# delldu/MaskRCNN

Measured on AMD Instinct MI355X. Metric: images/sec at 1024x1024, 1000 proposals/img (Mask R-CNN inference hot path), higher is better.
Workload: dtype f32

## Files before the change

include/maskrcnn_hip.h:

```cpp
#ifndef MASKRCNN_HIP_H
#define MASKRCNN_HIP_H

#include <stddef.h>
#include <stdint.h>

#ifdef __cplusplus
extern "C" {
#endif

#define MRCNN_ABI_VERSION 22

#define MRCNN_OK 0
#define MRCNN_ERR_INVALID_ARGUMENT (-1)
#define MRCNN_ERR_UNSUPPORTED (-2)
#define MRCNN_ERR_LAUNCH (-3)

typedef void* mrcnn_stream_t;

int mrcnn_abi_version(void);
const char* mrcnn_last_error(void);
const char* mrcnn_arch(void);

int64_t mrcnn_nms_max_boxes(void);
size_t mrcnn_nms_workspace_bytes(int32_t num_segments, int64_t n_max);
int mrcnn_nms_batched_f32(const float* dets, int32_t num_segments, int64_t n_max, int64_t seg_stride,
                          int64_t row_stride, int64_t col_stride, const int32_t* seg_counts,
                          const int32_t* class_ids, float threshold, int64_t* keep_out,
                          int32_t* counts_out, void* workspace, size_t workspace_bytes,
                          mrcnn_stream_t stream);

size_t mrcnn_nms_general_workspace_bytes(int64_t n, int32_t dtype);
int mrcnn_nms_general(const void* dets, int32_t dtype, int64_t n, int64_t row_stride, int64_t col_stride, float threshold,
                      int64_t* keep_out, int64_t* count_out, void* workspace, size_t workspace_bytes,
                      mrcnn_stream_t stream);

int mrcnn_crop_forward_f32(const float* image, int32_t batch, int32_t depth, int32_t height,
                           int32_t width, const float* boxes, const int32_t* box_index,
                           int32_t num_boxes, float extrapolation_value, int32_t crop_height,
                           int32_t crop_width, float* crops, mrcnn_stream_t stream);

int mrcnn_crop_backward_f32(const float* grads, const float* boxes, const int32_t* box_index,
                            int32_t num_boxes, int32_t batch, int32_t depth, int32_t height,
                            int32_t width, int32_t crop_height, int32_t crop_width,
// ... 133 lines not shown
int mrcnn_nhwc_to_kblocked_f32(const float* x, int64_t pixels, int32_t channels, float* y, mrcnn_stream_t stream);
size_t mrcnn_conv3x3_winograd_workspace_bytes(int32_t batch, int32_t height, int32_t width, int32_t cin);
int mrcnn_conv3x3_winograd_nhwc_f32(const float* x, int32_t batch, int32_t height, int32_t width, int32_t cin,
                                    const float* u, int32_t cout, const float* scale, const float* shift,
                                    int32_t activation, float* y, void* workspace, size_t workspace_bytes,
                                    mrcnn_stream_t stream);

int mrcnn_stem_conv7x7_s2_nhwc_f32(const float* x, int32_t batch, int32_t height, int32_t width, const float* w,
                                   const float* scale, const float* shift, int32_t activation, float* y,
                                   mrcnn_stream_t stream);
int mrcnn_stem_conv7x7_s2_nchw_f32(const float* x_nchw, int32_t batch, int32_t height, int32_t width, const float* w,
                                   const float* scale, const float* shift, int32_t activation, float* y,
                                   mrcnn_stream_t stream);
int mrcnn_stem_conv7x7_s2_nchw_f16out(const float* x_nchw, int32_t batch, int32_t height, int32_t width, const float* w,
                                      const float* scale, const float* shift, int32_t activation, void* y_f16,
                                      mrcnn_stream_t stream);
int mrcnn_stem_conv7x7_s2_pool_f32(const float* x_nchw, int32_t batch, int32_t height, int32_t width, const float* w,
                                   const float* scale, const float* shift, float* y, mrcnn_stream_t stream);
int mrcnn_stem_conv7x7_s2_pool_f16(const float* x_nchw, int32_t batch, int32_t height, int32_t width, const float* w,
                                   const float* scale, const float* shift, void* y_f16, mrcnn_stream_t stream);

size_t mrcnn_topk_workspace_bytes(int32_t batch);
int mrcnn_topk_desc_f32(const float* scores, int32_t batch, int64_t n, int32_t k, float* top_scores, int64_t* order,
                        void* workspace, size_t workspace_bytes, mrcnn_stream_t stream);
int mrcnn_proposal_select_f32(const float* dets, const int64_t* keep, const int32_t* keep_counts, int32_t batch,
                              int32_t k, int32_t proposal_count, float image_height, float image_width, float* rois,
                              int32_t* counts, mrcnn_stream_t stream);
int mrcnn_detection_select_f32(const float* dets, const int32_t* nms_class_ids, const int64_t* class_ids,
                               const int64_t* keep, const int32_t* keep_counts, int32_t batch, int32_t rois_per_image,
                               int32_t max_instances, float image_height, float image_width, int64_t* out_class_ids,
                               float* out_scores, float* out_boxes, float* out_rois, int32_t* out_counts,
                               mrcnn_stream_t stream);

int mrcnn_nchw_to_nhwc_f32(const float* x, int32_t batch, int32_t channels, int32_t height,
                           int32_t width, int32_t channels_padded, float* y, mrcnn_stream_t stream);
int mrcnn_nhwc_to_nchw_f32(const float* x, int32_t batch, int32_t channels, int32_t height,
                           int32_t width, float* y, mrcnn_stream_t stream);

size_t mrcnn_resize_u8_workspace_bytes(int32_t n, int32_t in_h, int32_t in_w, int32_t channels, int32_t out_h,
                                       int32_t out_w);
int mrcnn_resize_bilinear_u8(const uint8_t* src, int32_t n, int32_t in_h, int32_t in_w, int32_t channels,
                             int64_t src_image_stride, int64_t src_row_stride, uint8_t* dst, int32_t out_h,
                             int32_t out_w, void* workspace, size_t workspace_bytes, mrcnn_stream_t stream);
int mrcnn_mold_image_u8(const uint8_t* src, int32_t in_h, int32_t in_w, int32_t new_h, int32_t new_w, int32_t top,
                        int32_t left, int32_t out_h, int32_t out_w, const double mean_pixel[3], float* dst,
                        void* workspace, size_t workspace_bytes, mrcnn_stream_t stream);
int mrcnn_mold_images_u8(const uint8_t* src, int32_t n, int64_t src_image_stride, int32_t in_h, int32_t in_w, int32_t new_h,
                         int32_t new_w, int32_t top, int32_t left, int32_t out_h, int32_t out_w, const double mean_pixel[3],
                         float* dst, void* workspace, size_t workspace_bytes, mrcnn_stream_t stream);
int mrcnn_paste_masks_u8(const float* masks, int64_t stride_n, int64_t stride_y, int64_t stride_x, int64_t stride_c,
                         int32_t n, int32_t mask_h, int32_t mask_w, int32_t num_classes, const int64_t* class_ids,
                         const float* boxes, int32_t height, int32_t width, int32_t on_value, uint8_t* out,
                         mrcnn_stream_t stream);
size_t mrcnn_rle_workspace_bytes(int32_t n, int32_t height, int32_t width);
int mrcnn_rle_encode_u8(const uint8_t* masks, int64_t image_stride, int64_t row_stride, int32_t n, int32_t height,
                        int32_t width, int32_t threshold, int32_t capacity, int32_t* num_runs, uint32_t* counts,
                        uint8_t* strings, int32_t* string_bytes, int32_t* areas, int32_t* bboxes, void* workspace,
                        size_t workspace_bytes, mrcnn_stream_t stream);

size_t mrcnn_rle_iou_workspace_bytes(int32_t n_dt, int32_t dt_capacity, int32_t n_gt, int32_t gt_capacity);
int mrcnn_rle_iou_f64(const int32_t* dt_num_runs, const uint32_t* dt_counts, int32_t n_dt, int32_t dt_capacity,
                      const int32_t* gt_num_runs, const uint32_t* gt_counts, int32_t n_gt, int32_t gt_capacity,
                      const uint8_t* iscrowd, const int32_t* dt_off, const int32_t* gt_off, const int64_t* out_off,
                      int32_t groups, double* out, int64_t out_len, void* workspace, size_t workspace_bytes,
                      mrcnn_stream_t stream);
int mrcnn_bbox_iou_f64(const double* dt_boxes, int32_t n_dt, const double* gt_boxes, int32_t n_gt, const uint8_t* iscrowd,
// ... 59 lines not shown
```

maskrcnn_amd/csrc/common.hpp:

```cpp
#pragma once
#include <hip/hip_runtime.h>

#include <cstdarg>
#include <cstdint>
#include <cstdio>
#include <cstdlib>

#include "maskrcnn_hip.h"

namespace mrcnn {

char* error_buffer();
int fail(int code, const char* fmt, ...);

inline hipStream_t as_stream(mrcnn_stream_t s) { return reinterpret_cast<hipStream_t>(s); }

inline int check_launch(const char* what) {
    hipError_t e = hipGetLastError();
    if (e != hipSuccess) return fail(MRCNN_ERR_LAUNCH, "%s: %s", what, hipGetErrorString(e));
    return MRCNN_OK;
}

constexpr int kWave = 64;

int ensure_dynamic_lds(const void* kernel, size_t lds_bytes, const char* who);
int device_cu_count();

inline const char* tuning_env(const char* name) {
#ifdef MRCNN_TUNING
    return getenv(name);
#else
    (void)name;
    return nullptr;
#endif
}

}

#ifdef MRCNN_SYNC_FUZZ
namespace mrcnn {
__device__ __forceinline__ void sync_fuzz_point() {
    unsigned long long t;
    unsigned r;
    asm volatile("s_memtime %0\n\t"
                 "s_getreg_b32 %1, hwreg(HW_REG_HW_ID, 4, 2)\n\t"
                 "s_waitcnt lgkmcnt(0)\n\t"
                 "s_lshl_b32 %1, %1, 1\n\t"
                 "s_add_u32 %1, %1, 3\n\t"
                 "s_lshr_b64 %0, %0, %1\n\t"
                 "s_and_b64 %0, %0, 63\n\t"
                 "1:\n\t"
                 "s_cmp_eq_u64 %0, 0\n\t"
                 "s_cbranch_scc1 2f\n\t"
                 "s_sleep 64\n\t"
                 "s_lshr_b64 %0, %0, 1\n\t"
                 "s_branch 1b\n\t"
                 "2:"
                 : "=&s"(t), "=&s"(r)
                 :
                 : "scc", "memory");
}
__device__ __forceinline__ void fuzzed_syncthreads() {
    __syncthreads();
    sync_fuzz_point();
}
}
#define MRCNN_SYNC_FUZZ_POINT() ::mrcnn::sync_fuzz_point()
#define __syncthreads() ::mrcnn::fuzzed_syncthreads()
// ... 9 lines not shown
```

maskrcnn_amd/csrc/nms.hip:

```cpp
#pragma clang fp contract(off)

#include "common.hpp"

namespace {

using u64 = unsigned long long;
using u32 = unsigned int;

struct Box {
    float y1, x1, y2, x2, area;
};

__device__ __forceinline__ bool iou_ge(const Box& i, const Box& j, float thr) {
    const float xx1 = (i.x1 < j.x1) ? j.x1 : i.x1;
    const float yy1 = (i.y1 < j.y1) ? j.y1 : i.y1;
    const float xx2 = (j.x2 < i.x2) ? j.x2 : i.x2;
    const float yy2 = (j.y2 < i.y2) ? j.y2 : i.y2;
    float tw = xx2 - xx1;
    tw = tw + 1.0f;
    float th = yy2 - yy1;
    th = th + 1.0f;
    const float w = (0.0f < tw) ? tw : 0.0f;
    const float h = (0.0f < th) ? th : 0.0f;
    const float inter = w * h;
// ... 377 lines not shown
                       col_stride, seg_counts, class_ids, thr, keep_out, counts_out);
    return mrcnn::check_launch("nms_kernel");
}

template <int CAP, int T>
int launch_sort(const float* dets, int32_t S, int64_t n_max, int64_t seg_stride, int64_t row_stride,
                int64_t col_stride, const int32_t* seg_counts, const int32_t* class_ids, NmsWs ws,
                hipStream_t stream) {
    if (int rc = mrcnn::ensure_dynamic_lds(reinterpret_cast<const void*>(nms_sort_kernel<CAP, T>), sizeof(u64) * CAP, "nms"))
        return rc;
    hipLaunchKernelGGL((nms_sort_kernel<CAP, T>), dim3(S), dim3(T), sizeof(u64) * CAP, stream, dets, n_max,
                       seg_stride, row_stride, col_stride, seg_counts, class_ids, ws);
    return mrcnn::check_launch("nms_sort_kernel");
}

size_t ws_layout(int32_t S, int64_t n_max, void* base, NmsWs* ws) {
    const int np = static_cast<int>((n_max + 63) / 64 * 64), nb = np / 64;
    size_t off = 0;
    auto take = [&](size_t bytes) { size_t o = off; off += (bytes + 255) / 256 * 256; return o; };
    const size_t o_box = take(sizeof(float4) * S * np), o_area = take(sizeof(float) * S * np);
    const size_t o_cls = take(sizeof(int) * S * np), o_idx = take(sizeof(int) * S * np);
    const size_t o_col = take(sizeof(u64) * S * np * nb);
    if (ws) {
        unsigned char* b = static_cast<unsigned char*>(base);
        ws->box = reinterpret_cast<float4*>(b + o_box);
        ws->area = reinterpret_cast<float*>(b + o_area);
        ws->cls = reinterpret_cast<int*>(b + o_cls);
        ws->idx = reinterpret_cast<int*>(b + o_idx);
        ws->col = reinterpret_cast<u64*>(b + o_col);
        ws->np = np;
        ws->nb = nb;
    }
    return off;
}

}

constexpr int64_t NMS_MAX_WS = 16384, NMS_MAX_LDS = 4096;
extern "C" int64_t mrcnn_nms_max_boxes(void) { return NMS_MAX_WS; }

extern "C" size_t mrcnn_nms_workspace_bytes(int32_t num_segments, int64_t n_max) {
    if (num_segments < 1 || n_max < 1 || n_max > NMS_MAX_WS) return 0;
    return ws_layout(num_segments, n_max, nullptr, nullptr);
}

extern "C" int mrcnn_nms_batched_f32(const float* dets, int32_t num_segments, int64_t n_max,
                                     int64_t seg_stride, int64_t row_stride, int64_t col_stride,
                                     const int32_t* seg_counts, const int32_t* class_ids,
                                     float threshold, int64_t* keep_out, int32_t* counts_out,
                                     void* workspace, size_t workspace_bytes, mrcnn_stream_t stream) {
    MRCNN_REQUIRE(dets && keep_out && counts_out, "nms: null pointer");
    MRCNN_REQUIRE(num_segments >= 1, "nms: num_segments=%d must be >= 1", num_segments);
    MRCNN_REQUIRE(n_max >= 1 && n_max <= ((workspace && n_max > 128) ? NMS_MAX_WS : NMS_MAX_LDS),
                  "nms: n_max=%lld outside [1, %lld] (%lld with a workspace)", (long long)n_max, (long long)NMS_MAX_LDS,
                  (long long)NMS_MAX_WS);
    hipStream_t s = mrcnn::as_stream(stream);
    if (workspace && n_max > 128) {
        MRCNN_REQUIRE(workspace_bytes >= mrcnn_nms_workspace_bytes(num_segments, n_max),
                      "nms: workspace too small (%zu < %zu bytes)", workspace_bytes,
                      mrcnn_nms_workspace_bytes(num_segments, n_max));
        MRCNN_REQUIRE((reinterpret_cast<uintptr_t>(workspace) & 15) == 0, "nms: workspace must be 16-byte aligned");
        NmsWs ws;
        ws_layout(num_segments, n_max, workspace, &ws);
        int rc;
        if (n_max <= 1024)
            rc = launch_sort<1024, 1024>(dets, num_segments, n_max, seg_stride, row_stride, col_stride,
// ... 9 lines not shown
                                         seg_counts, class_ids, ws, s);
        else
            rc = launch_sort<16384, 1024>(dets, num_segments, n_max, seg_stride, row_stride, col_stride,
                                          seg_counts, class_ids, ws, s);
        if (rc) return rc;
        hipLaunchKernelGGL(nms_mask_kernel, dim3(ws.nb * (ws.nb + 1) / 2, num_segments), dim3(64), 0, s, ws,
                           threshold);
        if ((rc = mrcnn::check_launch("nms_mask_kernel"))) return rc;
        const size_t tail = (ws.np + 7) / 8 * 8 + sizeof(u64) * (ws.nb + 2);
        const size_t lds_full = sizeof(u64) * ws.np * ws.nb + tail;
        if (lds_full <= 150 * 1024) {
            auto k = nms_scan_kernel<true>;
            if ((rc = mrcnn::ensure_dynamic_lds(reinterpret_cast<const void*>(k), lds_full, "nms"))) return rc;
            hipLaunchKernelGGL(k, dim3(num_segments), dim3(256), lds_full, s, ws, n_max, seg_counts, keep_out,
                               counts_out);
        } else {
            hipLaunchKernelGGL(nms_scan_kernel<false>, dim3(num_segments), dim3(256), tail, s, ws, n_max,
                               seg_counts, keep_out, counts_out);
        }
        return mrcnn::check_launch("nms_scan_kernel");
    }
    if (n_max <= 256)
        return launch<256, 256>(dets, num_segments, n_max, seg_stride, row_stride, col_stride,
                                seg_counts, class_ids, threshold, keep_out, counts_out, s);
    if (n_max <= 1024)
        return launch<1024, 1024>(dets, num_segments, n_max, seg_stride, row_stride, col_stride,
                                  seg_counts, class_ids, threshold, keep_out, counts_out, s);
    if (n_max <= 2048)
        return launch<2048, 1024>(dets, num_segments, n_max, seg_stride, row_stride, col_stride,
                                  seg_counts, class_ids, threshold, keep_out, counts_out, s);
    return launch<4096, 1024>(dets, num_segments, n_max, seg_stride, row_stride, col_stride,
                              seg_counts, class_ids, threshold, keep_out, counts_out, s);
}
```

maskrcnn_amd/csrc/select.hip:

```cpp
#include "common.hpp"

namespace {

constexpr int TOPK_THREADS = 1024;
constexpr int TOPK_WAVES = TOPK_THREADS / 64;
constexpr int SORT_CAP = 4096;

__device__ __forceinline__ uint32_t order_key(float f) {
    uint32_t u = __float_as_uint(f);
    if (f != f) u = 0x7FC00000u;
    return (u & 0x80000000u) ? ~u : (u | 0x80000000u);
}

template <typename T>
__device__ __forceinline__ void bitonic_sort_desc(T* keys, int n, int tid, int nthreads) {
    for (int k = 2; k <= n; k <<= 1) {
        for (int j = k >> 1; j > 0; j >>= 1) {
            __syncthreads();
            for (int i = tid; i < n; i += nthreads) {
                const int l = i ^ j;
                if (l > i) {
                    const T a = keys[i], b = keys[l];
                    const bool desc = (i & k) == 0;
                    if (desc ? a < b : a > b) {
// ... 398 lines not shown
        float score = 0.f;
        int64_t id = 0;
        if (ok) {
            const uint32_t idx = 0xFFFFFFFFu - static_cast<uint32_t>(e);
            box = make_float4(db[idx * 5 + 0], db[idx * 5 + 1], db[idx * 5 + 2], db[idx * 5 + 3]);
            score = db[idx * 5 + 4];
            id = class_ids[static_cast<int64_t>(b) * p + idx];
        }
        out_ids[o] = id;
        out_scores[o] = score;
        reinterpret_cast<float4*>(out_boxes)[o] = box;
        reinterpret_cast<float4*>(out_rois)[o] =
            make_float4(box.x / norm_h, box.y / norm_w, box.z / norm_h, box.w / norm_w);
        return ok;
    };
    int cnt = 0;
    if (p <= 1024) {
        const uint64_t v = sort1024_desc(key_of(tid), sh.keys, tid);
        if (tid < d) cnt += emit(tid, v);
    } else {
        for (int i = tid; i < pp; i += 1024) sh.keys[i] = key_of(i);
        bitonic_sort_desc(sh.keys, pp, tid, 1024);
        for (int i = tid; i < d; i += 1024) cnt += emit(i, sh.keys[i]);
    }
    __syncthreads();
    uint32_t* total = sh.kept;
    if (tid == 0) total[0] = 0;
    __syncthreads();
    if (cnt) atomicAdd(&total[0], static_cast<uint32_t>(cnt));
    __syncthreads();
    if (tid == 0) out_counts[b] = static_cast<int32_t>(total[0]);
}

}

static size_t topk_layout(int batch, TopkWorkspace* ws, unsigned char* base) {
    auto up = [](size_t v) { return (v + 255) & ~static_cast<size_t>(255); };
    size_t o = 0;
    const size_t counters = o; o += up(sizeof(uint32_t) * 2 * batch);
    const size_t maxima = o;   o += up(sizeof(uint32_t) * static_cast<size_t>(batch) * TOPK_NMAX);
    const size_t cand = o;     o += up(sizeof(uint64_t) * static_cast<size_t>(batch) * SORT_CAP);
    if (ws) {
        uint32_t* c = reinterpret_cast<uint32_t*>(base + counters);
        ws->ncand = c;
        ws->bound = c + batch;
        ws->maxima = reinterpret_cast<uint32_t*>(base + maxima);
        ws->cand = reinterpret_cast<uint64_t*>(base + cand);
    }
    return o;
}

extern "C" size_t mrcnn_topk_workspace_bytes(int32_t batch) {
    return batch >= 1 ? topk_layout(batch, nullptr, nullptr) : 0;
}

extern "C" int mrcnn_topk_desc_f32(const float* scores, int32_t batch, int64_t n, int32_t k, float* top_scores,
                                   int64_t* order, void* workspace, size_t workspace_bytes, mrcnn_stream_t stream) {
    MRCNN_REQUIRE(scores && top_scores && order && workspace, "topk: null pointer");
    MRCNN_REQUIRE(batch >= 1 && batch <= 65535 && n >= 1 && n < (1LL << 32) - 1, "topk: batch=%d n=%lld", batch,
                  static_cast<long long>(n));
    MRCNN_REQUIRE(k >= 1 && k <= SORT_CAP && k <= n, "topk: k=%d must be in [1, min(n, %d)]", k, SORT_CAP);
    TopkWorkspace ws;
    const size_t need = topk_layout(batch, &ws, static_cast<unsigned char*>(workspace));
    MRCNN_REQUIRE(workspace_bytes >= need, "topk: workspace too small (%zu < %zu)", workspace_bytes, need);
    hipStream_t s = mrcnn::as_stream(stream);
    hipLaunchKernelGGL(topk_maxima_kernel, dim3(TOPK_SPLIT, batch), dim3(TOPK_THREADS), 0, s, scores, n, ws);
// ... 3 lines not shown
    return mrcnn::check_launch("topk kernels");
}

extern "C" int mrcnn_proposal_select_f32(const float* dets, const int64_t* keep, const int32_t* keep_counts,
                                         int32_t batch, int32_t k, int32_t proposal_count, float image_height,
                                         float image_width, float* rois, int32_t* counts, mrcnn_stream_t stream) {
    MRCNN_REQUIRE(dets && keep && keep_counts && rois && counts, "proposal_select: null pointer");
    MRCNN_REQUIRE(batch >= 1 && batch <= 65535 && k >= 1 && proposal_count >= 1 && proposal_count <= k,
                  "proposal_select: batch=%d k=%d proposal_count=%d (1 <= proposal_count <= k)", batch, k,
                  proposal_count);
    hipLaunchKernelGGL(proposal_select_kernel, dim3((proposal_count + 255) / 256, batch), dim3(256), 0,
                       mrcnn::as_stream(stream), dets, keep, keep_counts, k, proposal_count, image_height, image_width,
                       rois, counts);
    return mrcnn::check_launch("proposal_select_kernel");
}

extern "C" int mrcnn_detection_select_f32(const float* dets, const int32_t* nms_class_ids, const int64_t* class_ids,
                                          const int64_t* keep, const int32_t* keep_counts, int32_t batch,
                                          int32_t rois_per_image, int32_t max_instances, float image_height,
                                          float image_width, int64_t* out_class_ids, float* out_scores,
                                          float* out_boxes, float* out_rois, int32_t* out_counts,
                                          mrcnn_stream_t stream) {
    MRCNN_REQUIRE(dets && nms_class_ids && class_ids && keep && keep_counts && out_class_ids && out_scores &&
                      out_boxes && out_rois && out_counts, "detection_select: null pointer");
    MRCNN_REQUIRE(batch >= 1 && rois_per_image >= 1 && rois_per_image <= SORT_CAP,
                  "detection_select: batch=%d rois_per_image=%d (<= %d)", batch, rois_per_image, SORT_CAP);
    MRCNN_REQUIRE(max_instances >= 1 && max_instances <= rois_per_image,
                  "detection_select: max_instances=%d must be in [1, rois_per_image]", max_instances);
    hipLaunchKernelGGL(detection_select_kernel, dim3(batch), dim3(1024), 0, mrcnn::as_stream(stream), dets,
                       nms_class_ids, class_ids, keep, keep_counts, rois_per_image, max_instances, image_height,
                       image_width, out_class_ids, out_scores, out_boxes, out_rois, out_counts);
    return mrcnn::check_launch("detection_select_kernel");
}
```

maskrcnn_amd/ops.py:

```python
from __future__ import annotations

import ctypes
import functools
import math
import os
import weakref

import numpy as np
import torch

from ._lib import MaskrcnnHipError, c_f32, c_i32, c_vp, check, lib

__all__ = ["nms_batched", "nms_general", "crop", "roi_align_pyramid", "MaskrcnnHipError",
           "conv_bn_act", "conv_bn_act_f16mfma", "split_f16", "same_pad", "maxpool", "nchw_to_nhwc", "nhwc_to_nchw",
           "bottleneck_forward", "bottleneck_fused", "bottleneck_fused_supported", "bottleneck_native", "bottleneck_plan",
           "rpn_scores_deltas", "proposal_decode", "conv3x3_winograd_heads", "HeadSums",
           "detection_decode", "topk_desc", "proposal_select", "detection_select", "deconv2x2", "rpn_level_fused",
           "rle_encode", "rle_iou", "bbox_iou", "coco_match", "rle_from_poly", "rle_merge",
           "rle_from_string", "rle_area_bbox", "rle_to_string", "rle_decode"]

_LIB = torch.library.Library("maskrcnn", "DEF")


def _stream() -> int:
    return torch.cuda.current_stream().cuda_stream


def _ptr(t):
    return None if t is None else t.data_ptr()


class HeadSums:

    def __init__(self, part: torch.Tensor, batch: int, height: int, width: int, tile_mode: int = 1):
        self.part, self.batch, self.height, self.width, self.tile_mode = part, batch, height, width, tile_mode

    def to_nhwc(self, bias: torch.Tensor) -> torch.Tensor:
        b, h, w = self.batch, self.height, self.width
        if self.tile_mode == 4:
            return ((self.part[0, :, :18] + self.part[1, :, :18]) + bias).view(b, h, w, 18).contiguous()
        th, tw = h // 2, w // 2
        if self.tile_mode == 1:
            t = b * th * tw
            v = (self.part[0, :t * 4, :18] + self.part[1, :t * 4, :18]) + bias
            return v.view(b, th, tw, 2, 2, 18).permute(0, 1, 3, 2, 4, 5).reshape(b, h, w, 18).contiguous()
        if self.tile_mode == 3:
            tyb, txb = -(-(h // 4) // 4), -(-(w // 4) // 8)
            v = self.part[:, :18] + bias
            v = v.view(b, tyb, txb, 4, 8, 4, 4, 18).permute(0, 1, 3, 5, 2, 4, 6, 7).reshape(b, tyb * 16, txb * 32, 18)
            return v[:, :h, :w].contiguous()
# ... 794 lines not shown
    _need_gpu(dets, keep, keep_counts)
    assert dets.is_contiguous() and keep.is_contiguous() and keep.dtype == torch.int64
    assert keep_counts.dtype == torch.int32 and keep_counts.is_contiguous()
    b, k, _ = dets.shape
    rois = torch.empty(b, proposal_count, 4, dtype=torch.float32, device=dets.device)
    counts = torch.empty(b, dtype=torch.int32, device=dets.device)
    check(lib.mrcnn_proposal_select_f32(dets.data_ptr(), keep.data_ptr(), keep_counts.data_ptr(), b, k,
                                        proposal_count, float(image_height), float(image_width), rois.data_ptr(),
                                        counts.data_ptr(), _stream()))
    return rois, counts


@_on_device
def detection_select(dets, nms_class_ids, class_ids, keep, keep_counts, max_instances: int, image_height,
                     image_width):
    _need_gpu(dets, nms_class_ids, class_ids, keep, keep_counts)
    assert dets.is_contiguous() and nms_class_ids.is_contiguous() and class_ids.is_contiguous()
    assert keep.is_contiguous() and keep.dtype == torch.int64 and class_ids.dtype == torch.int64
    assert nms_class_ids.dtype == torch.int32 and keep_counts.dtype == torch.int32
    b, p, _ = dets.shape
    d, dev = max_instances, dets.device
    ids = torch.empty(b, d, dtype=torch.int64, device=dev)
    scores = torch.empty(b, d, dtype=torch.float32, device=dev)
    boxes = torch.empty(b, d, 4, dtype=torch.float32, device=dev)
    rois = torch.empty(b, d, 4, dtype=torch.float32, device=dev)
    counts = torch.empty(b, dtype=torch.int32, device=dev)
    check(lib.mrcnn_detection_select_f32(dets.data_ptr(), nms_class_ids.data_ptr(), class_ids.data_ptr(),
                                         keep.data_ptr(), keep_counts.data_ptr(), b, p, d, float(image_height),
                                         float(image_width), ids.data_ptr(), scores.data_ptr(), boxes.data_ptr(),
                                         rois.data_ptr(), counts.data_ptr(), _stream()))
    return ids, scores, boxes, rois, counts


@_on_device
def deconv2x2(x: torch.Tensor, w, bias4: torch.Tensor, activation: int = 0, products: int = 0) -> torch.Tensor:
    _need_gpu(x, bias4)
    assert x.is_contiguous() and x.dtype in (torch.float32, torch.float16) and bias4.is_contiguous()
    b, h, wd, cin = x.shape
    w0 = w if products == 0 else w[0]
    cout = w0.size(0) // 4
    assert w0.size(3) == cin and bias4.numel() == 4 * cout
    y = torch.empty(b, 2 * h, 2 * wd, cout, dtype=x.dtype, device=x.device)

    def book():
        m = b * h * wd
        return (2.0 * m * cin * 4 * cout, (m, 4 * cout, cin),
                x.element_size() * (x.numel() + y.numel()) + (4 if products == 0 else 2 * (2 if products == 3 else 1)) * w0.numel(),
                "direct" if products == 0 else "f16")
    if products == 0:
        assert w.dtype == torch.float32 and w.is_contiguous()
        _launch(lib.mrcnn_deconv2x2_bias_act_nhwc_f32,
                (x.data_ptr(), b, h, wd, cin, w.data_ptr(), cout, bias4.data_ptr(), int(activation), y.data_ptr(), _stream()), book)
    elif x.dtype == torch.float16:
        assert products == 1
        _launch(lib.mrcnn_deconv2x2_bias_act_nhwc_f16io,
                (x.data_ptr(), b, h, wd, cin, w[0].data_ptr(), cout, bias4.data_ptr(), int(activation), y.data_ptr(), _stream()),
                book)
    else:
        w_hi, w_lo = w
        _launch(lib.mrcnn_deconv2x2_bias_act_nhwc_f16mfma,
                (x.data_ptr(), b, h, wd, cin, w_hi.data_ptr(), _ptr(w_lo), cout, bias4.data_ptr(), int(activation), int(products),
                 y.data_ptr(), _stream()), book)
    return y


HAVE_ABLATIONS = hasattr(lib, "mrcnn_rpn_level_fused_f32")
# ... 740 lines not shown
```

maskrcnn_amd/pipeline.py:

```python
from __future__ import annotations

import os
from dataclasses import dataclass

import torch

from . import image as imagelib
from . import modules, ops
from .anchors import pyramid_anchors
from .config import InferenceConfig


@dataclass
class Detections:
    class_ids: torch.Tensor
    scores: torch.Tensor
    boxes: torch.Tensor
    counts: torch.Tensor
    masks: torch.Tensor | None

    def packed(self) -> torch.Tensor:
        return torch.cat([self.class_ids.float().unsqueeze(-1), self.scores.unsqueeze(-1), self.boxes], -1)


# ... 15 lines not shown
    return max(1, n)


class MaskRCNNInference:
    def __init__(self, state_dict: dict, cfg: InferenceConfig | None = None, device="cuda:0",
                 precision: str = "f32", concurrent_sub_batches: int | None = None):
        assert precision in modules.PRECISIONS + (modules.MIXED,), precision
        self.cfg = cfg or InferenceConfig()
        self.precision = precision
        self.device = torch.device(device)
        if self.device.type != "cuda":
            raise RuntimeError("MaskRCNNInference runs on the GPU only (no CPU path)")
        c = self.cfg
        self.backbone = modules.FusedBackbone(state_dict, c.backbone, self.device, precision=precision)
        self.rpn = modules.FusedRPN(state_dict, self.device, precision=precision)
        self.classifier = modules.FusedClassifier(state_dict, self.device, precision=precision)
        self.mask = modules.FusedMask(state_dict, self.device, precision=precision)
        self.anchors = pyramid_anchors(c).to(self.device)
        self.image_area = float(c.image_height * c.image_width)
        self.max_batch = max_batch_per_launch(c, precision)
        env = os.environ.get("MRCNN_SUB_BATCHES")
        self.sub_batches = int(env) if env else (concurrent_sub_batches if concurrent_sub_batches is not None
                                                  else (2 if precision == "f16" else 1))
        self._side_streams, self._keep, self._keep_event = [], None, None

    def rpn_heads(self, fms):
        kb = getattr(self.backbone, "kblocked", None) or [None] * len(fms)
        return ops.rpn_scores_deltas([self.rpn(p, k) for p, k in zip(fms, kb)], self.rpn.b_head)

    def proposals(self, scores, deltas):
        c = self.cfg
        k = min(c.pre_nms_limit, self.anchors.size(0))
        top, order = ops.topk_desc(scores, k)
        dets = ops.proposal_decode(self.anchors, deltas, order, top, c.rpn_bbox_std_dev, c.image_height,
                                   c.image_width)
        keep, kept = ops.nms_batched(dets, c.rpn_nms_threshold)
        rois, counts = ops.proposal_select(dets, keep, kept, min(c.proposal_count, k), c.image_height,
                                           c.image_width)
        return rois, counts, dets

    def detections(self, rois, roi_counts, logits, bbox, windows):
        c = self.cfg
        p = rois.size(1)
        dets, cls, class_ids = ops.detection_decode(logits, bbox, rois.contiguous(), roi_counts,
                                                    windows.to(torch.float32).contiguous(), c.rpn_bbox_std_dev,
                                                    c.image_height, c.image_width,
                                                    float(c.detection_min_confidence or 0.0))
        keep, kept = ops.nms_batched(dets, c.detection_nms_threshold, class_ids=cls)
        return ops.detection_select(dets, cls, class_ids, keep, kept, min(c.detection_max_instances, p),
                                    c.image_height, c.image_width)

    @torch.no_grad()
    def predict(self, images: torch.Tensor, windows: torch.Tensor, with_masks: bool = True,
                return_intermediates: bool = False, rois_override=None, host_counts=None, _whole: bool = False):
        c = self.cfg
        assert images.is_cuda and images.dtype == torch.float32
        b = images.size(0)
        assert tuple(images.shape[1:]) == (3, c.image_height, c.image_width)
        if b > self.max_batch:
            assert not return_intermediates, f"return_intermediates needs batch <= {self.max_batch} at this image size"
            assert host_counts is None, "host_counts: one launch group per call (batch <= max_batch)"
            n = -(-b // self.max_batch)
            step = -(-b // n)
            ro = rois_override
            parts = [self.predict(images[i:i + step], windows[i:i + step], with_masks,
                                  rois_override=None if ro is None else (ro[0][i:i + step], ro[1][i:i + step]))
                     for i in range(0, b, step)]
            cat = lambda f: torch.cat([getattr(p_, f) for p_ in parts], 0)
            return Detections(cat("class_ids"), cat("scores"), cat("boxes"), cat("counts"), cat("masks") if with_masks else None)
        k = self.sub_batches
        if (k > 1 and not _whole and b >= k and b % k == 0 and not return_intermediates and host_counts is None
                and ops.CONV_PROFILE is None
                and not torch.cuda.is_current_stream_capturing()):
            return self._predict_concurrent(images, windows, with_masks, rois_override, k)
        fms = self.backbone(images)
        scores, deltas = self.rpn_heads(fms)
        rois, roi_counts, rpn_dets = self.proposals(scores, deltas)
        if rois_override is not None:
            o_rois, o_counts = rois_override
            assert tuple(o_rois.shape) == tuple(rois.shape) and o_rois.dtype == torch.float32 and o_rois.is_cuda
# ... 140 lines not shown
```

Before: 421.4.

## Fuse proposal decode with NMS sort/mask and NMS scan with selection

Adds a kernel that decodes proposals, checks order and bitonic-sorts in LDS, then writes NMS workspace directly before launching the IoU mask kernel. A second kernel pair runs the NMS suppression scan in LDS inside the proposal and detection selection kernels, so the separate keep and count buffers and extra launches go away. This applies when boxes per image fall in (128, 1024]. The scan runs serially in one wave per image, and the LDS needed for the column mask grows with the segment size, which may limit occupancy.

```diff
diff --git a/include/maskrcnn_hip.h b/include/maskrcnn_hip.h
--- a/include/maskrcnn_hip.h
+++ b/include/maskrcnn_hip.h
@@ -8,7 +8,7 @@
 extern "C" {
 #endif
 
-#define MRCNN_ABI_VERSION 22
+#define MRCNN_ABI_VERSION 23
 
 #define MRCNN_OK 0
 #define MRCNN_ERR_INVALID_ARGUMENT (-1)
@@ -208,6 +208,26 @@
                                float* out_scores, float* out_boxes, float* out_rois, int32_t* out_counts,
                                mrcnn_stream_t stream);
 
+int mrcnn_proposal_decode_nms_mask_f32(const float* anchors, const float* deltas, const int64_t* order,
+                                       const float* top_scores, const int32_t* seg_counts, int32_t batch,
+                                       int32_t num_anchors, int32_t k, const float std_dev[4], float image_height,
+                                       float image_width, float threshold, float* dets, void* workspace,
+                                       size_t workspace_bytes, mrcnn_stream_t stream);
+int mrcnn_nms_order_mask_f32(const float* dets, int32_t num_segments, int64_t n_max, int64_t seg_stride,
+                             int64_t row_stride, int64_t col_stride, const int32_t* seg_counts,
+                             const int32_t* class_ids, float threshold, void* workspace, size_t workspace_bytes,
+                             mrcnn_stream_t stream);
+int mrcnn_nms_scan_proposal_select_f32(const float* dets, const int32_t* seg_counts, int32_t batch, int32_t k,
+                                       int32_t proposal_count, float image_height, float image_width,
+                                       const void* workspace, size_t workspace_bytes, float* rois, int32_t* counts,
+                                       mrcnn_stream_t stream);
+int mrcnn_nms_scan_detection_select_f32(const float* dets, const int32_t* nms_class_ids, const int64_t* class_ids,
+                                        const int32_t* seg_counts, int32_t batch, int32_t rois_per_image,
+                                        int32_t max_instances, float image_height, float image_width,
+                                        const void* workspace, size_t workspace_bytes, int64_t* out_class_ids,
+                                        float* out_scores, float* out_boxes, float* out_rois, int32_t* out_counts,
+                                        mrcnn_stream_t stream);
+
 int mrcnn_nchw_to_nhwc_f32(const float* x, int32_t batch, int32_t channels, int32_t height,
                            int32_t width, int32_t channels_padded, float* y, mrcnn_stream_t stream);
 int mrcnn_nhwc_to_nchw_f32(const float* x, int32_t batch, int32_t channels, int32_t height,
diff --git a/maskrcnn_amd/csrc/common.hpp b/maskrcnn_amd/csrc/common.hpp
--- a/maskrcnn_amd/csrc/common.hpp
+++ b/maskrcnn_amd/csrc/common.hpp
@@ -34,6 +34,13 @@
     return nullptr;
 #endif
 }
+
+struct NmsScanView {
+    const int* idx;
+    const unsigned long long* col;
+    int np, nb;
+};
+size_t nms_scan_view(int32_t num_segments, int64_t n_max, void* workspace, NmsScanView* view);
 
 }
 
diff --git a/maskrcnn_amd/csrc/nms.hip b/maskrcnn_amd/csrc/nms.hip
--- a/maskrcnn_amd/csrc/nms.hip
+++ b/maskrcnn_amd/csrc/nms.hip
@@ -433,6 +433,105 @@
         ws->nb = nb;
     }
     return off;
+}
+
+__device__ __forceinline__ float4 refine_clamp(const float4 an, const float4 dl, float s0, float s1, float s2, float s3,
+                                               float img_h, float img_w) {
+    const float dy = dl.x * s0, dx = dl.y * s1, dh = dl.z * s2, dw = dl.w * s3;
+    float height = an.z - an.x;
+    float width = an.w - an.y;
+    float cy = an.x + 0.5f * height;
+    float cx = an.y + 0.5f * width;
+    cy = cy + dy * height;
+    cx = cx + dx * width;
+    height = height * expf(dh);
+    width = width * expf(dw);
+    float y1 = cy - 0.5f * height;
+    float x1 = cx - 0.5f * width;
+    float y2 = y1 + height;
+    float x2 = x1 + width;
+    y1 = fminf(fmaxf(y1, 0.f), img_h);
+    x1 = fminf(fmaxf(x1, 0.f), img_w);
+    y2 = fminf(fmaxf(y2, 0.f), img_h);
+    x2 = fminf(fmaxf(x2, 0.f), img_w);
+    return make_float4(y1, x1, y2, x2);
+}
+
+__global__ __launch_bounds__(1024) void proposal_decode_order_kernel(
+    const float* __restrict__ anchors, const float* __restrict__ deltas, const int64_t* __restrict__ order,
+    const float* __restrict__ top_scores, const int32_t* __restrict__ seg_counts, int A, int K, float s0, float s1, float s2,
+    float s3, float img_h, float img_w, float* __restrict__ dets, NmsWs ws) {
+    constexpr int T = 1024;
+    __shared__ u64 keys[T];
+    __shared__ float4 sbox[T];
+    __shared__ int unsorted;
+    const int seg = blockIdx.x, tid = threadIdx.x;
+    int n = seg_counts ? seg_counts[seg] : K;
+    n = n < 0 ? 0 : (n > K ? K : n);
+    int np2 = 64;
+    while (np2 < n) np2 <<= 1;
+    float4 box = make_float4(0.f, 0.f, 0.f, 0.f);
+    u64 key = ~0ull;
+    if (tid < K) {
+        const int64_t e = static_cast<int64_t>(seg) * K + tid;
+        const int64_t idx = order[e];
+        const float4 an = *reinterpret_cast<const float4*>(anchors + idx * 4);
+        const float4 dl = *reinterpret_cast<const float4*>(deltas + (static_cast<int64_t>(seg) * A + idx) * 4);
+        box = refine_clamp(an, dl, s0, s1, s2, s3, img_h, img_w);
+        const float score = top_scores[e];
+        float* o = dets + e * 5;
+        o[0] = box.x; o[1] = box.y; o[2] = box.z; o[3] = box.w; o[4] = score;
+        if (tid < n) key = make_key(score, static_cast<u32>(tid));
+    }
+    keys[tid] = key;
+    sbox[tid] = box;
+    if (tid == 0) unsorted = 0;
+    __syncthreads();
+    if (tid + 1 < n && keys[tid] > keys[tid + 1]) unsorted = 1;
+    __syncthreads();
+    int idx = tid < n ? tid : -1;
+    if (unsorted) {
+        for (int k = 2; k <= np2; k <<= 1) {
+            for (int j = k >> 1; j > 0; j >>= 1) {
+                for (int t = tid; t < (np2 >> 1); t += T) {
+                    const int i = ((t & ~(j - 1)) << 1) | (t & (j - 1));
+                    const u64 a = keys[i], b = keys[i + j];
+                    const bool up = (i & k) == 0;
+                    if ((a > b) == up) {
+                        keys[i] = b;
+                        keys[i + j] = a;
+                    }
+                }
+                __syncthreads();
+            }
+        }
+        if (tid < n) {
+            idx = static_cast<int>(keys[tid] & 0xFFFFFFFFu);
+            box = sbox[idx];
+        }
+    }
+    if (tid < ws.np) {
+        float area = 0.f;
+        if (tid < n) {
+            float w = box.w - box.y;
+            w = w + 1.0f;
+            float h = box.z - box.x;
+            h = h + 1.0f;
+            area = w * h;
+        } else {
+            box = make_float4(0.f, 0.f, 0.f, 0.f);
+        }
+        const int64_t base = static_cast<int64_t>(seg) * ws.np;
+        ws.box[base + tid] = box;
+        ws.area[base + tid] = area;
+        ws.cls[base + tid] = 0;
+        ws.idx[base + tid] = idx;
+    }
+}
+
+int launch_mask(const NmsWs& ws, int32_t num_segments, float threshold, hipStream_t s) {
+    hipLaunchKernelGGL(nms_mask_kernel, dim3(ws.nb * (ws.nb + 1) / 2, num_segments), dim3(64), 0, s, ws, threshold);
+    return mrcnn::check_launch("nms_mask_kernel");
 }
 
 }
@@ -508,3 +607,62 @@
     return launch<4096, 1024>(dets, num_segments, n_max, seg_stride, row_stride, col_stride,
                               seg_counts, class_ids, threshold, keep_out, counts_out, s);
 }
+
+constexpr int64_t NMS_MAX_FUSED = 1024;
+
+size_t mrcnn::nms_scan_view(int32_t num_segments, int64_t n_max, void* workspace, mrcnn::NmsScanView* view) {
+    NmsWs ws;
+    const size_t bytes = ws_layout(num_segments, n_max, workspace, &ws);
+    if (view) {
+        view->idx = ws.idx;
+        view->col = ws.col;
+        view->np = ws.np;
+        view->nb = ws.nb;
+    }
+    return bytes;
+}
+
+extern "C" int mrcnn_proposal_decode_nms_mask_f32(const float* anchors, const float* deltas, const int64_t* order,
+                                                  const float* top_scores, const int32_t* seg_counts, int32_t batch,
+                                                  int32_t num_anchors, int32_t k, const float std_dev[4],
+                                                  float image_height, float image_width, float threshold, float* dets,
+                                                  void* workspace, size_t workspace_bytes, mrcnn_stream_t stream) {
+    MRCNN_REQUIRE(anchors && deltas && order && top_scores && std_dev && dets && workspace,
+                  "proposal_decode_nms_mask: null pointer");
+    MRCNN_REQUIRE(batch >= 1 && num_anchors >= 1, "proposal_decode_nms_mask: bad sizes");
+    MRCNN_REQUIRE(k >= 1 && k <= NMS_MAX_FUSED, "proposal_decode_nms_mask: k=%d outside [1, %lld]", k,
+                  (long long)NMS_MAX_FUSED);
+    MRCNN_REQUIRE(workspace_bytes >= mrcnn_nms_workspace_bytes(batch, k),
+                  "proposal_decode_nms_mask: workspace too small (%zu < %zu bytes)", workspace_bytes,
+                  mrcnn_nms_workspace_bytes(batch, k));
+    MRCNN_REQUIRE((reinterpret_cast<uintptr_t>(workspace) & 15) == 0, "proposal_decode_nms_mask: workspace must be 16-byte aligned");
+    hipStream_t s = mrcnn::as_stream(stream);
+    NmsWs ws;
+    ws_layout(batch, k, workspace, &ws);
+    hipLaunchKernelGGL(proposal_decode_order_kernel, dim3(batch), dim3(1024), 0, s, anchors, deltas, order, top_scores,
+                       seg_counts, num_anchors, k, std_dev[0], std_dev[1], std_dev[2], std_dev[3], image_height,
+                       image_width, dets, ws);
+    if (int rc = mrcnn::check_launch("proposal_decode_order_kernel")) return rc;
+    return launch_mask(ws, batch, threshold, s);
+}
+
+extern "C" int mrcnn_nms_order_mask_f32(const float* dets, int32_t num_segments, int64_t n_max, int64_t seg_stride,
+                                        int64_t row_stride, int64_t col_stride, const int32_t* seg_counts,
+                                        const int32_t* class_ids, float threshold, void* workspace,
+                                        size_t workspace_bytes, mrcnn_stream_t stream) {
+    MRCNN_REQUIRE(dets && workspace, "nms_order_mask: null pointer");
+    MRCNN_REQUIRE(num_segments >= 1, "nms_order_mask: num_segments=%d must be >= 1", num_segments);
+    MRCNN_REQUIRE(n_max >= 1 && n_max <= NMS_MAX_FUSED, "nms_order_mask: n_max=%lld outside [1, %lld]", (long long)n_max,
+                  (long long)NMS_MAX_FUSED);
+    MRCNN_REQUIRE(workspace_bytes >= mrcnn_nms_workspace_bytes(num_segments, n_max),
+                  "nms_order_mask: workspace too small (%zu < %zu bytes)", workspace_bytes,
+                  mrcnn_nms_workspace_bytes(num_segments, n_max));
+    MRCNN_REQUIRE((reinterpret_cast<uintptr_t>(workspace) & 15) == 0, "nms_order_mask: workspace must be 16-byte aligned");
+    hipStream_t s = mrcnn::as_stream(stream);
+    NmsWs ws;
+    ws_layout(num_segments, n_max, workspace, &ws);
+    if (int rc = launch_sort<1024, 1024>(dets, num_segments, n_max, seg_stride, row_stride, col_stride, seg_counts,
+                                         class_ids, ws, s))
+        return rc;
+    return launch_mask(ws, num_segments, threshold, s);
+}
diff --git a/maskrcnn_amd/csrc/select.hip b/maskrcnn_amd/csrc/select.hip
--- a/maskrcnn_amd/csrc/select.hip
+++ b/maskrcnn_amd/csrc/select.hip
@@ -454,6 +454,132 @@
     if (tid == 0) out_counts[b] = static_cast<int32_t>(total[0]);
 }
 
+using u64 = unsigned long long;
+constexpr int SCAN_THREADS = 1024;
+
+__host__ __device__ inline size_t scan_lds_bytes(int np, int nb) { return sizeof(u64) * np * nb + np + sizeof(u64) * (nb + 2); }
+
+__device__ __forceinline__ void nms_scan_flags(const mrcnn::NmsScanView& ws, int seg, int n, unsigned char* smem,
+                                               unsigned char*& keepf) {
+    const int tid = threadIdx.x, lane = tid & 63, wave = tid >> 6;
+    const int np = ws.np, nb = ws.nb;
+    const int64_t base = static_cast<int64_t>(seg) * np;
+    const u64* gcol = ws.col + base * nb;
+    u64* lcol = reinterpret_cast<u64*>(smem);
+    keepf = smem + sizeof(u64) * np * nb;
+    u64* keptw = reinterpret_cast<u64*>(keepf + np);
+    const int nchunks = (n + 63) >> 6;
+    for (int rb = 0; rb < nchunks; ++rb)
+        for (int p = rb * 64 + tid; p < nchunks * 64; p += SCAN_THREADS) lcol[rb * np + p] = gcol[static_cast<int64_t>(rb) * np + p];
+    for (int i = tid; i < np; i += SCAN_THREADS) keepf[i] = 0;
+    __syncthreads();
+    const u64* ck = lcol;
+    if (wave == 0) {
+        for (int c = 0; c < nchunks; ++c) {
+            const int p = c * 64 + lane;
+            const u64 dc = ck[static_cast<int64_t>(c) * np + p];
+            u64 rem = 0;
+            int rb = 0;
+            for (; rb + 8 <= c; rb += 8) {
+                u64 v[8];
+#pragma unroll
+                for (int u = 0; u < 8; ++u) v[u] = ck[static_cast<int64_t>(rb + u) * np + p];
+#pragma unroll
+                for (int u = 0; u < 8; ++u) rem |= v[u] & keptw[rb + u];
+            }
+            for (; rb < c; ++rb) rem |= ck[static_cast<int64_t>(rb) * np + p] & keptw[rb];
+            const bool me_alive = p < n && rem == 0ull;
+            u64 kept = __ballot(me_alive);
+            for (int round = 0; round < 65; ++round) {
+                const u64 next = __ballot(me_alive && (dc & kept) == 0ull);
+                if (next == kept) break;
+                kept = next;
+            }
+            if (lane == 0) keptw[c] = kept;
+        }
+    }
+    __syncthreads();
+    for (int p = tid; p < n; p += SCAN_THREADS)
+        if ((keptw[p >> 6] >> (p & 63)) & 1ull) keepf[ws.idx[base + p]] = 1;
+    __syncthreads();
+}
+
+__device__ __forceinline__ int segment_count(const int32_t* __restrict__ seg_counts, int seg, int n_max) {
+    const int n = seg_counts ? seg_counts[seg] : n_max;
+    return n < 0 ? 0 : (n > n_max ? n_max : n);
+}
+
+__global__ __launch_bounds__(SCAN_THREADS) void nms_scan_proposal_select_kernel(
+    mrcnn::NmsScanView ws, const float* __restrict__ dets, const int32_t* __restrict__ seg_counts, int k, int p, float norm_h,
+    float norm_w, float* __restrict__ rois, int32_t* __restrict__ counts) {
+    extern __shared__ __attribute__((aligned(16))) unsigned char smem[];
+    __shared__ int wave_sum[SCAN_THREADS / 64];
+    const int b = blockIdx.x, tid = threadIdx.x, lane = tid & 63, wave = tid >> 6;
+    const int n = segment_count(seg_counts, b, k);
+    unsigned char* keepf;
+    nms_scan_flags(ws, b, n, smem, keepf);
+    const bool f = tid < n && keepf[tid];
+    const u64 m = __ballot(f);
+    if (lane == 0) wave_sum[wave] = __popcll(m);
+    __syncthreads();
+    int before = 0, total = 0;
+    for (int w = 0; w < SCAN_THREADS / 64; ++w) {
+        const int v = wave_sum[w];
+        before += w < wave ? v : 0;
+        total += v;
+    }
+    const int cnt = min(total, p);
+    const int pos = before + __popcll(m & ((1ull << lane) - 1ull));
+    float4* out = reinterpret_cast<float4*>(rois) + static_cast<int64_t>(b) * p;
+    if (f && pos < p) {
+        const float* d = dets + (static_cast<int64_t>(b) * k + tid) * 5;
+        out[pos] = make_float4(d[0] / norm_h, d[1] / norm_w, d[2] / norm_h, d[3] / norm_w);
+    }
+    if (tid >= cnt && tid < p) out[tid] = make_float4(0.f, 0.f, 0.f, 0.f);
+    if (tid == 0) counts[b] = cnt;
+}
+
+__global__ __launch_bounds__(SCAN_THREADS) void nms_scan_detection_select_kernel(
+    mrcnn::NmsScanView ws, const float* __restrict__ dets, const int32_t* __restrict__ nms_cls,
+    const int64_t* __restrict__ class_ids, const int32_t* __restrict__ seg_counts, int p, int d, float norm_h, float norm_w,
+    int64_t* __restrict__ out_ids, float* __restrict__ out_scores, float* __restrict__ out_boxes, float* __restrict__ out_rois,
+    int32_t* __restrict__ out_counts) {
+    extern __shared__ __attribute__((aligned(16))) unsigned char smem[];
+    __shared__ uint64_t sortbuf[2 * 1024];
+    __shared__ uint32_t total;
+    const int b = blockIdx.x, tid = threadIdx.x;
+    const float* db = dets + static_cast<int64_t>(b) * p * 5;
+    const int n = segment_count(seg_counts, b, p);
+    unsigned char* keepf;
+    nms_scan_flags(ws, b, n, smem, keepf);
+    uint64_t key = 0;
+    if (tid < p && keepf[tid] && nms_cls[static_cast<int64_t>(b) * p + tid] > 0)
+        key = (static_cast<uint64_t>(order_key(db[tid * 5 + 4])) << 32) | (0xFFFFFFFFu - static_cast<uint32_t>(tid));
+    if (tid == 0) total = 0;
+    const uint64_t e = sort1024_desc(key, sortbuf, tid);
+    const bool ok = e != 0;
+    if (tid < d) {
+        const int64_t o = static_cast<int64_t>(b) * d + tid;
+        float4 box = make_float4(0.f, 0.f, 0.f, 0.f);
+        float score = 0.f;
+        int64_t id = 0;
+        if (ok) {
+            const uint32_t idx = 0xFFFFFFFFu - static_cast<uint32_t>(e);
+            box = make_float4(db[idx * 5 + 0], db[idx * 5 + 1], db[idx * 5 + 2], db[idx * 5 + 3]);
+            score = db[idx * 5 + 4];
+            id = class_ids[static_cast<int64_t>(b) * p + idx];
+        }
+        out_ids[o] = id;
+        out_scores[o] = score;
+        reinterpret_cast<float4*>(out_boxes)[o] = box;
+        reinterpret_cast<float4*>(out_rois)[o] =
+            make_float4(box.x / norm_h, box.y / norm_w, box.z / norm_h, box.w / norm_w);
+        if (ok) atomicAdd(&total, 1u);
+    }
+    __syncthreads();
+    if (tid == 0) out_counts[b] = static_cast<int32_t>(total);
+}
+
 }
 
 static size_t topk_layout(int batch, TopkWorkspace* ws, unsigned char* base) {
@@ -523,3 +649,50 @@
                        image_width, out_class_ids, out_scores, out_boxes, out_rois, out_counts);
     return mrcnn::check_launch("detection_select_kernel");
 }
+
+constexpr int SCAN_SELECT_MAX = 1024;
+
+extern "C" int mrcnn_nms_scan_proposal_select_f32(const float* dets, const int32_t* seg_counts, int32_t batch, int32_t k,
+                                                  int32_t proposal_count, float image_height, float image_width,
+                                                  const void* workspace, size_t workspace_bytes, float* rois,
+                                                  int32_t* counts, mrcnn_stream_t stream) {
+    MRCNN_REQUIRE(dets && workspace && rois && counts, "nms_scan_proposal_select: null pointer");
+    MRCNN_REQUIRE(batch >= 1 && batch <= 65535 && k >= 1 && k <= SCAN_SELECT_MAX && proposal_count >= 1 && proposal_count <= k,
+                  "nms_scan_proposal_select: batch=%d k=%d proposal_count=%d (1 <= proposal_count <= k <= %d)", batch, k,
+                  proposal_count, SCAN_SELECT_MAX);
+    mrcnn::NmsScanView ws;
+    const size_t need = mrcnn::nms_scan_view(batch, k, const_cast<void*>(workspace), &ws);
+    MRCNN_REQUIRE(workspace_bytes >= need, "nms_scan_proposal_select: workspace too small (%zu < %zu bytes)", workspace_bytes,
+                  need);
+    const size_t lds = scan_lds_bytes(ws.np, ws.nb);
+    auto kern = nms_scan_proposal_select_kernel;
+    if (int rc = mrcnn::ensure_dynamic_lds(reinterpret_cast<const void*>(kern), lds, "nms_scan_proposal_select")) return rc;
+    hipLaunchKernelGGL(kern, dim3(batch), dim3(SCAN_THREADS), lds, mrcnn::as_stream(stream), ws, dets, seg_counts, k,
+                       proposal_count, image_height, image_width, rois, counts);
+    return mrcnn::check_launch("nms_scan_proposal_select_kernel");
+}
+
+extern "C" int mrcnn_nms_scan_detection_select_f32(const float* dets, const int32_t* nms_class_ids, const int64_t* class_ids,
+                                                   const int32_t* seg_counts, int32_t batch, int32_t rois_per_image,
+                                                   int32_t max_instances, float image_height, float image_width,
+                                                   const void* workspace, size_t workspace_bytes, int64_t* out_class_ids,
+                                                   float* out_scores, float* out_boxes, float* out_rois,
+                                                   int32_t* out_counts, mrcnn_stream_t stream) {
+    MRCNN_REQUIRE(dets && nms_class_ids && class_ids && workspace && out_class_ids && out_scores && out_boxes && out_rois &&
+                      out_counts, "nms_scan_detection_select: null pointer");
+    MRCNN_REQUIRE(batch >= 1 && batch <= 65535 && rois_per_image >= 1 && rois_per_image <= SCAN_SELECT_MAX,
+                  "nms_scan_detection_select: batch=%d rois_per_image=%d (<= %d)", batch, rois_per_image, SCAN_SELECT_MAX);
+    MRCNN_REQUIRE(max_instances >= 1 && max_instances <= rois_per_image,
+                  "nms_scan_detection_select: max_instances=%d must be in [1, rois_per_image]", max_instances);
+    mrcnn::NmsScanView ws;
+    const size_t need = mrcnn::nms_scan_view(batch, rois_per_image, const_cast<void*>(workspace), &ws);
+    MRCNN_REQUIRE(workspace_bytes >= need, "nms_scan_detection_select: workspace too small (%zu < %zu bytes)",
+                  workspace_bytes, need);
+    const size_t lds = scan_lds_bytes(ws.np, ws.nb);
+    auto kern = nms_scan_detection_select_kernel;
+    if (int rc = mrcnn::ensure_dynamic_lds(reinterpret_cast<const void*>(kern), lds, "nms_scan_detection_select")) return rc;
+    hipLaunchKernelGGL(kern, dim3(batch), dim3(SCAN_THREADS), lds, mrcnn::as_stream(stream), ws, dets, nms_class_ids,
+                       class_ids, seg_counts, rois_per_image, max_instances, image_height, image_width, out_class_ids,
+                       out_scores, out_boxes, out_rois, out_counts);
+    return mrcnn::check_launch("nms_scan_detection_select_kernel");
+}
diff --git a/maskrcnn_amd/ops.py b/maskrcnn_amd/ops.py
--- a/maskrcnn_amd/ops.py
+++ b/maskrcnn_amd/ops.py
@@ -16,6 +16,7 @@
            "bottleneck_forward", "bottleneck_fused", "bottleneck_fused_supported", "bottleneck_native", "bottleneck_plan",
            "rpn_scores_deltas", "proposal_decode", "conv3x3_winograd_heads", "HeadSums",
            "detection_decode", "topk_desc", "proposal_select", "detection_select", "deconv2x2", "rpn_level_fused",
+           "proposals_fused", "detections_fused", "select_fused_supported",
            "rle_encode", "rle_iou", "bbox_iou", "coco_match", "rle_from_poly", "rle_merge",
            "rle_from_string", "rle_area_bbox", "rle_to_string", "rle_decode"]
 
@@ -876,6 +877,71 @@
     return ids, scores, boxes, rois, counts
 
 
+SELECT_FUSED_MAX = 1024
+
+
+def select_fused_supported(boxes_per_image: int) -> bool:
+    return 128 < boxes_per_image <= SELECT_FUSED_MAX
+
+
+def _nms_workspace(s: int, n: int, device):
+    nbytes = int(lib.mrcnn_nms_workspace_bytes(s, n))
+    return torch.empty(nbytes, dtype=torch.uint8, device=device), nbytes
+
+
+@_on_device
+def proposals_fused(anchors, deltas, order, top_scores, std_dev, image_height, image_width, threshold: float,
+                    proposal_count: int, seg_counts: torch.Tensor | None = None):
+    _need_gpu(anchors, deltas, order, top_scores, seg_counts)
+    assert anchors.is_contiguous() and deltas.is_contiguous() and order.is_contiguous() and top_scores.is_contiguous()
+    assert order.dtype == torch.int64 and deltas.dtype == torch.float32 and top_scores.dtype == torch.float32
+    b, k = order.shape
+    assert 1 <= proposal_count <= k <= SELECT_FUSED_MAX
+    if seg_counts is not None:
+        assert seg_counts.dtype == torch.int32 and seg_counts.is_contiguous() and seg_counts.numel() == b
+    dev = deltas.device
+    dets = torch.empty(b, k, 5, dtype=torch.float32, device=dev)
+    rois = torch.empty(b, proposal_count, 4, dtype=torch.float32, device=dev)
+    counts = torch.empty(b, dtype=torch.int32, device=dev)
+    ws, ws_bytes = _nms_workspace(b, k, dev)
+    check(lib.mrcnn_proposal_decode_nms_mask_f32(anchors.data_ptr(), deltas.data_ptr(), order.data_ptr(),
+                                                 top_scores.data_ptr(), _ptr(seg_counts), b, anchors.size(0), k,
+                                                 (c_f32 * 4)(*[float(v) for v in std_dev]), float(image_height),
+                                                 float(image_width), float(threshold), dets.data_ptr(), ws.data_ptr(),
+                                                 ws_bytes, _stream()))
+    check(lib.mrcnn_nms_scan_proposal_select_f32(dets.data_ptr(), _ptr(seg_counts), b, k, proposal_count,
+                                                 float(image_height), float(image_width), ws.data_ptr(), ws_bytes,
+                                                 rois.data_ptr(), counts.data_ptr(), _stream()))
+    return rois, counts, dets
+
+
+@_on_device
+def detections_fused(dets, nms_class_ids, class_ids, threshold: float, max_instances: int, image_height, image_width,
+                     seg_counts: torch.Tensor | None = None):
+    _need_gpu(dets, nms_class_ids, class_ids, seg_counts)
+    assert dets.is_contiguous() and dets.dtype == torch.float32 and nms_class_ids.is_contiguous() and class_ids.is_contiguous()
+    assert class_ids.dtype == torch.int64 and nms_class_ids.dtype == torch.int32
+    b, p, _ = dets.shape
+    assert 1 <= max_instances <= p <= SELECT_FUSED_MAX and nms_class_ids.numel() == b * p and class_ids.numel() == b * p
+    if seg_counts is not None:
+        assert seg_counts.dtype == torch.int32 and seg_counts.is_contiguous() and seg_counts.numel() == b
+    d, dev = max_instances, dets.device
+    ids = torch.empty(b, d, dtype=torch.int64, device=dev)
+    scores = torch.empty(b, d, dtype=torch.float32, device=dev)
+    boxes = torch.empty(b, d, 4, dtype=torch.float32, device=dev)
+    rois = torch.empty(b, d, 4, dtype=torch.float32, device=dev)
+    counts = torch.empty(b, dtype=torch.int32, device=dev)
+    ws, ws_bytes = _nms_workspace(b, p, dev)
+    check(lib.mrcnn_nms_order_mask_f32(dets.data_ptr(), b, p, dets.stride(0), dets.stride(1), dets.stride(2),
+                                       _ptr(seg_counts), nms_class_ids.data_ptr(), float(threshold), ws.data_ptr(), ws_bytes,
+                                       _stream()))
+    check(lib.mrcnn_nms_scan_detection_select_f32(dets.data_ptr(), nms_class_ids.data_ptr(), class_ids.data_ptr(),
+                                                  _ptr(seg_counts), b, p, d, float(image_height), float(image_width),
+                                                  ws.data_ptr(), ws_bytes, ids.data_ptr(), scores.data_ptr(),
+                                                  boxes.data_ptr(), rois.data_ptr(), counts.data_ptr(), _stream()))
+    return ids, scores, boxes, rois, counts
+
+
 @_on_device
 def deconv2x2(x: torch.Tensor, w, bias4: torch.Tensor, activation: int = 0, products: int = 0) -> torch.Tensor:
     _need_gpu(x, bias4)
diff --git a/maskrcnn_amd/pipeline.py b/maskrcnn_amd/pipeline.py
--- a/maskrcnn_amd/pipeline.py
+++ b/maskrcnn_amd/pipeline.py
@@ -71,6 +71,9 @@
         c = self.cfg
         k = min(c.pre_nms_limit, self.anchors.size(0))
         top, order = ops.topk_desc(scores, k)
+        if ops.select_fused_supported(k):
+            return ops.proposals_fused(self.anchors, deltas, order, top, c.rpn_bbox_std_dev, c.image_height, c.image_width,
+                                       c.rpn_nms_threshold, min(c.proposal_count, k))
         dets = ops.proposal_decode(self.anchors, deltas, order, top, c.rpn_bbox_std_dev, c.image_height,
                                    c.image_width)
         keep, kept = ops.nms_batched(dets, c.rpn_nms_threshold)
@@ -85,6 +88,9 @@
                                                     windows.to(torch.float32).contiguous(), c.rpn_bbox_std_dev,
                                                     c.image_height, c.image_width,
                                                     float(c.detection_min_confidence or 0.0))
+        if ops.select_fused_supported(p):
+            return ops.detections_fused(dets, cls, class_ids, c.detection_nms_threshold, min(c.detection_max_instances, p),
+                                        c.image_height, c.image_width)
         keep, kept = ops.nms_batched(dets, c.detection_nms_threshold, class_ids=cls)
         return ops.detection_select(dets, cls, class_ids, keep, kept, min(c.detection_max_instances, p),
                                     c.image_height, c.image_width)
```

Result: no change. 421.2 (-0.1%).
